# Thefefe/orbit

Hardware: AMD Instinct MI355X
Metric: meshlets_culled_per_sec (higher is better)
Workload: dtype f32

## Files before the change

orbit_amd/csrc/abi_ctx.hip:

```cpp
#include <cstdarg>
#include <cstdio>
#include <cstdlib>

#include "abi_internal.h"

thread_local char g_err[512] = "no error";

int32_t fail(OrbitCtx *ctx, int32_t code, const char *fmt, ...) {
    char buf[512];
    va_list ap;
    va_start(ap, fmt);
    vsnprintf(buf, sizeof(buf), fmt, ap);
    va_end(ap);
    snprintf(g_err, sizeof(g_err), "%s", buf);
    if (ctx) snprintf(ctx->err, sizeof(ctx->err), "%s", buf);
    return code;
}

namespace {

size_t layout_arena(OrbitCtx *ctx, uintptr_t base, uint64_t md32) {
    const OrbitCaps &caps = ctx->caps;
    const size_t ent = align_up((size_t)caps.max_entities, 256);
    const size_t mtiles = ((size_t)md32 + kTileRecords - 1) / kTileRecords + 1;
    const size_t cchunks = ((size_t)caps.max_clusters / 1024 + 64) * 32;
    size_t off = 0;
    auto carve = [&](size_t bytes) {
        const uintptr_t p = base + off;
        off = align_up(off + bytes, 256);
        return p;
    };
    ctx->status = (int32_t *)carve(256);
    ctx->debug_cycles = (unsigned long long *)carve(256 + 16 * 8192);
    ctx->zero_page = (void *)carve(256);
    ctx->g_counts = (uint32_t *)carve(256);
    ctx->m_tickets = (uint32_t *)carve((kTicketPools + kEmitTicketPools) * kTicketStride * 4);
    ctx->m_list_sync = (uint32_t *)carve(kListSyncWords * 4);
    ctx->f_done = (uint32_t *)carve((size_t)kShardDoneWords * kShardDoneStride * 4);
    ctx->f_sync = (uint32_t *)carve(kFusedSyncWords * 4);
    ctx->f_ent_flags = (uint32_t *)carve((ent / 256 + 2) * 4);
    ctx->d_tickets = (uint32_t *)carve((size_t)kMaxPyramidBatch * kDepthTicketWords * 4);
    ctx->e_proto = (OrbitMeshletDispatch *)carve(ent * sizeof(OrbitMeshletDispatch));
    ctx->e_block_sums = (uint32_t *)carve((ent / 256 + 1) * 4);
    ctx->e_total = (uint32_t *)carve(256);
    ctx->m_tile_counts = (uint32_t *)carve(mtiles * 4);
    ctx->m_tile_base = (uint32_t *)carve(mtiles * 4);
    ctx->m_total = (uint32_t *)carve(256);
    ctx->f_tile_flags = (uint32_t *)carve(((size_t)md32 / 4 + 2) * 4);
    ctx->m_split = ctx->rec_shift > 5u ? (uint8_t *)carve(ORBIT_DISPATCH_HEADER + 16 * (size_t)md32) : nullptr;
    ctx->x_block_pop = (uint32_t *)carve((size_t)kExpandBlocks * 4);
    ctx->m_tile_masks = (uint32_t *)carve(mtiles * 64);
    ctx->m_tile_payload = (Payload *)carve(mtiles * 128 * sizeof(Payload));
    ctx->m_chunk_sums = (uint32_t *)carve((mtiles / kScanChunk + 2) * 4);
    ctx->c_chunk = (uint32_t *)carve((2 * cchunks + 64) * 4);
    ctx->c_chunk_words = cchunks;
    ctx->a_view_lights = (float4 *)carve((size_t)caps.max_lights * 16 + 1024);
    ctx->a_light_flags = (uint32_t *)carve(((size_t)caps.max_lights / 32 + 64) * 4);
    ctx->a_counts = (uint32_t *)carve(((size_t)caps.max_clusters + kAssignPad) * 4);
    ctx->a_block_sums = (uint32_t *)carve((((size_t)caps.max_clusters / kScanChunk + 2) * kChunkSumStride + 64) * 4);
    ctx->a_block_base = (uint32_t *)carve(((size_t)caps.max_clusters + kAssignPad) * 4);
    ctx->a_total = (uint32_t *)carve(256);
    const size_t agroups = (size_t)caps.max_clusters / 256 + 1;
    const size_t aseg = (((size_t)caps.max_lights + 15) / 16 + 63) / 64 * 64;
    ctx->a_aabb = (float *)carve(((size_t)caps.max_clusters + kAssignPad) * 6 * 4);
    ctx->a_coarse = (uint32_t *)carve(agroups * 16 * aseg * 4);
    ctx->a_coarse_lights = (float4 *)carve(agroups * 16 * aseg * 16);
    ctx->a_coarse_counts = (uint32_t *)carve(agroups * 16 * 4);
    ctx->a_group_box = (float *)carve(agroups * 32);
    ctx->a_group_order = (uint32_t *)carve((agroups + 1) * 4);
    ctx->a_coarse_seg = (uint32_t)aseg;
    ctx->a_hit_cache = (uint32_t *)carve(((size_t)caps.max_clusters + kAssignPad) * kHitCache * 4);
// ... 254 lines not shown
```

orbit_amd/csrc/abi_cull.hip:

```cpp
#include "abi_internal.h"

namespace {

int32_t check_cull_info(OrbitCtx *ctx, const OrbitGpuCullInfo *ci) {
    if (!ci) return fail(ctx, ORBIT_E_INVALID, "cull_info is NULL");
    if (ci->cull_plane_count > ORBIT_MAX_CULL_PLANES)
        return fail(ctx, ORBIT_E_PLANES, "cull_plane_count %u > %d", ci->cull_plane_count, ORBIT_MAX_CULL_PLANES);
    if (ci->projection_type > 1) return fail(ctx, ORBIT_E_INVALID, "projection_type %u", ci->projection_type);
    if (ci->occlusion_pass > 2) return fail(ctx, ORBIT_E_INVALID, "occlusion_pass %u", ci->occlusion_pass);
    return ORBIT_OK;
}

MeshSideView mesh_side_for(OrbitMeshletStream *ms, const void *mesh_info_buffer, bool count = true) {
    if (!ms) return MeshSideView{nullptr, 0u};
    std::lock_guard<std::mutex> lock(ms->mu);
    if (ms->mesh_side == nullptr || ms->mesh_source != mesh_info_buffer || ms->mesh_hi == 0u) return MeshSideView{nullptr, 0u};
    if (count) ms->mesh_side_culls++;
    return MeshSideView{ms->mesh_side, ms->mesh_hi};
}

PyramidView make_pyramid_view(const float *texels, const uint32_t size[2],
                              const OrbitDepthPyramidLevel *levels = nullptr) {
    PyramidView v;
    v.texels = texels;
// ... 349 lines not shown
    PreparedCullViews pc;
    const int32_t rc = prepare_cull_views(ctx, views, count, 0u, pc);
    if (rc != ORBIT_OK) return rc;
    return launch_prepared_cull_views(ctx, pc, (hipStream_t)stream);
}

int32_t orbit_cull_shard(OrbitCtx *ctx, const OrbitGpuCullInfo *ci, const OrbitEntityCullBufs *eb, uint32_t draw_first,
                         uint32_t draw_count, const OrbitMeshletCullBufs *mb, void *record_buffer,
                         uint32_t record_capacity, uint32_t with_commands, void *stream) {
    if (!ctx) return fail(nullptr, ORBIT_E_INVALID, "ctx is NULL");
    std::lock_guard<std::mutex> lock(ctx->mu);
    if (ctx->rec_shift != 5u)
        return fail(ctx, ORBIT_E_INVALID, "cull_shard: the sharded engine's record list is defined for dispatch_size 32; this "
                                          "context has %u", ctx->caps.dispatch_size);
    const hipStream_t s = (hipStream_t)stream;
    const MeshletCullOut out{MeshletCullOut::kRecordList, record_buffer, record_capacity, with_commands ? "cull_shard" : nullptr};
    EntityCullParams ep;
    MeshletCullParams p;
    int32_t rc = entity_cull_params(ctx, ctx, ci, eb, draw_first, draw_count, true, ep);
    if (rc == ORBIT_OK) rc = meshlet_cull_params(ctx, ctx, ci, mb, out, p);
    if (rc != ORBIT_OK) return rc;
    if (mb->meshlet_dispatch_buffer != eb->meshlet_dispatch_buffer)
        return fail(ctx, ORBIT_E_INVALID, "cull_shard: the meshlet stage must read the entity stage's dispatch buffer");
    hipEvent_t ev0, ev1;
    rc = profile_pair(ctx, ev0, ev1);
    if (rc == ORBIT_OK) rc = validate_stream(ctx, p, s);
    if (rc == ORBIT_OK) rc = validate_mesh_side(ctx, ep, s);
    if (rc != ORBIT_OK) return rc;
    const uint32_t chunks = (draw_count + 255u) / 256u;
    const bool one_launch = ci->occlusion_pass == 0u && chunks >= 1u && chunks <= kShardMaxChunks && ctx->caps.cull_path != 1u;
    hipError_t e;
    if (one_launch) {
        FusedCullParams f = fused_params(ep, p, ctx, chunks);
        f.done_flags = ctx->f_done;
        if (ev0 && (e = hipEventRecord(ev0, s)) != hipSuccess) return hip_fail(ctx, e, "hipEventRecord");
        e = launch_shard_cull(f, ctx->num_cus, s);
        if (e != hipSuccess) return hip_fail(ctx, e, "launch shard_cull");
        if (ev1 && (e = hipEventRecord(ev1, s)) != hipSuccess) return hip_fail(ctx, e, "hipEventRecord");
        if (with_commands) {
            MeshletCullParams c = p;
            c.visible_list = 0u;
            c.draw_buffer = p.also_commands;
            c.draw_capacity = p.also_commands_capacity;
            e = launch_meshlet_scan_emit(c, ctx->num_cus, s);
            if (e != hipSuccess) return hip_fail(ctx, e, "launch scan + emit");
        }
        ctx->shard_culls++;
    } else {
        e = launch_entity_cull(ep, draw_count, ctx->num_cus, s);
        if (e != hipSuccess) return hip_fail(ctx, e, "launch entity_cull");
        e = launch_meshlet_cull(p, ctx->num_cus, s, ev0, ev1);
        if (e != hipSuccess) return hip_fail(ctx, e, "launch meshlet_cull");
    }
    count_stream_cull(ctx, p);
    return ORBIT_OK;
}

int32_t orbit_expand_visible_records(OrbitCtx *ctx, const void *record_buffer, const void *meshlet_buffer,
                                     void *draw_commands_buffer, uint32_t draw_capacity, void *stream) {
    if (!ctx) return fail(nullptr, ORBIT_E_INVALID, "ctx is NULL");
    std::lock_guard<std::mutex> lock(ctx->mu);
    if (!record_buffer || !meshlet_buffer || !draw_commands_buffer)
        return fail(ctx, ORBIT_E_MISSING, "expand_visible_records: NULL argument");
    const MeshletStreamView view = stream_view_for(ctx->meshlet_stream, meshlet_buffer, nullptr);
    if (view.sphere && ctx->caps.validate_streams)
        (void)launch_meshlet_stream_validate((const OrbitMeshlet *)meshlet_buffer, view, nullptr, 0, ctx->status,
                                             (hipStream_t)stream);
// ... 71 lines not shown
```

orbit_amd/csrc/abi_internal.h:

```cpp
#pragma once
#include <hip/hip_runtime.h>

#include <atomic>
#include <cstdint>
#include <cstring>
#include <mutex>
#include <new>
#include <vector>

#include "kernels.h"

using namespace orbit;

#pragma GCC visibility push(hidden)

struct OrbitMeshletStream {
    int device = 0;
    uint64_t first = 0, capacity = 0;
    uint4 *sphere = nullptr;
    uint32_t *cone = nullptr;
    uint16_t *mat = nullptr;
    uint32_t *cmd = nullptr;
    uint16_t *cnt = nullptr;
    uint32_t *link = nullptr, *cls0 = nullptr, *cls1 = nullptr;
// ... 7 lines not shown
    hipEvent_t other_event = nullptr;
    bool other_pending = false;
    bool other_recorded = false;
    std::atomic<int> bindings{0};
    MeshSide *mesh_side = nullptr;
    uint32_t mesh_capacity = 0, mesh_hi = 0;
    const void *mesh_source = nullptr;
    uint64_t mesh_side_culls = 0;
};

struct OrbitCtx {
    int device = 0;
    uint32_t num_cus = 0;
    OrbitCaps caps{};
    std::mutex mu;
    uint8_t *arena = nullptr;
    size_t arena_bytes = 0;
    OrbitMeshletDispatch *e_proto = nullptr;
    uint32_t *e_block_sums = nullptr, *e_total = nullptr;
    Payload *m_tile_payload = nullptr;
    uint32_t *m_tile_masks = nullptr, *m_chunk_sums = nullptr;
    uint32_t *m_tile_counts = nullptr, *m_tile_base = nullptr, *m_total = nullptr;
    uint32_t *s_block_sums = nullptr;
    float *b_mesh_slices = nullptr;
    uint32_t *x_block_pop = nullptr;
    uint32_t *c_chunk = nullptr;
    size_t c_chunk_words = 0;
    float4 *a_view_lights = nullptr, *a_coarse_lights = nullptr;
    uint32_t *a_light_flags = nullptr, *a_counts = nullptr, *a_block_sums = nullptr, *a_block_base = nullptr,
             *a_total = nullptr, *a_coarse = nullptr, *a_coarse_counts = nullptr, *a_hit_cache = nullptr;
    float *a_aabb = nullptr, *a_group_box = nullptr;
    uint32_t *a_group_order = nullptr;
    uint32_t a_coarse_seg = 0;
    uint32_t *m_tickets = nullptr, *m_list_sync = nullptr, *f_done = nullptr;
    uint32_t *f_sync = nullptr, *f_ent_flags = nullptr, *f_tile_flags = nullptr;
    uint32_t *d_tickets = nullptr;
    uint8_t *m_split = nullptr;
    uint32_t rec_shift = 5;
    uint64_t fused_culls = 0;
    uint64_t shard_culls = 0;
    uint32_t *g_counts = nullptr;
    int32_t *status = nullptr;
    uint32_t debug_flags = 0;
    uint32_t scan_patience = 256;
    unsigned long long *debug_cycles = nullptr;
    void *zero_page = nullptr;
    uint32_t profiling = 0;
    uint32_t prof_calls = 0;
    std::vector<hipEvent_t> prof_events;
    size_t prof_used = 0;
    std::vector<OrbitCtx *> view_ctx;
    hipStream_t side_stream[2] = {nullptr, nullptr};
    hipEvent_t side_event[3] = {nullptr, nullptr, nullptr};
    OrbitMeshletStream *meshlet_stream = nullptr;
    uint64_t stream_culls = 0;
    uint64_t class_culls = 0;
    char err[512] = {0};
};

constexpr uint32_t kExpandBlocks = 65536;

constexpr uint32_t kMeshBoundsSlots = 1024;

extern thread_local char g_err[512];

int32_t fail(OrbitCtx *ctx, int32_t code, const char *fmt, ...);

// ... 68 lines not shown
```

orbit_amd/csrc/entity_common.h:

```cpp
#pragma once
#include "handoff.h"

namespace orbit {

namespace {

constexpr int kEntityBlock = 256;

enum : uint32_t { kEntNone = 0, kEntSkipped, kEntFrustum, kEntOcclusion, kEntEarly, kEntDrawn };
struct EntityVerdict {
    uint32_t cls;
    uint32_t lod;
};

template <class P>
__device__ __forceinline__ OrbitMeshletDispatch entity_eval_one(const P &p, uint32_t g, bool active, bool &visible,
                                                                EntityVerdict *verdict = nullptr) {
    const OrbitGpuCullInfo &ci = p.ci;
    const bool meshlet_occ = ci.meshlet_visibility_buffer != ORBIT_NONE;
    visible = false;
    OrbitMeshletDispatch pr = {0u, 0u, 0u, 0u};
    if (verdict) verdict->cls = kEntNone, verdict->lod = 0u;
    if (active) {
        const OrbitEntityDraw *draws =
// ... 105 lines not shown
                const uint32_t mid = (lo[u] + hi[u]) >> 1;
                if (s_off[mid] <= r0 + u * kEntityBlock) lo[u] = mid; else hi[u] = mid;
            }
        }
#pragma unroll
        for (uint32_t u = 0; u < U; u++) {
            const uint32_t r = r0 + u * kEntityBlock;
            if (r < total) store(r, entity_record(s_proto[lo[u]], r - s_off[lo[u]], rec_shift));
        }
    }
}
static_assert(kEntityBlock == 256, "entity_expand_records: eight bisection steps");

struct FusedEntity {
    const OrbitGpuCullInfo &ci;
    const uint8_t *entity_draw_buffer;
    const OrbitMeshInfo *mesh_infos;
    MeshSideView mesh_side;
    const OrbitEntityData *entities;
    uint32_t *visibility;
    PyramidView pyr;
};

struct EntityChunksArgs {
    uint8_t *dispatch_buffer;
    uint32_t dispatch_capacity;
    uint32_t draw_first, draw_limit;
    uint32_t ne_chunks;
    uint32_t rec_shift;
    uint32_t *sync;
    uint32_t *ent_flags;
    uint32_t *total;
    int32_t *status;
};
struct EntityChunksLds {
    uint32_t smem[kEntityBlock / 64 + 1];
    uint32_t off[kEntityBlock];
    OrbitMeshletDispatch proto[kEntityBlock];
    uint32_t word;
};

__device__ __forceinline__ uint32_t chunks_before(int32_t *status, __amdgpu_buffer_rsrc_t EF, uint32_t eb, uint32_t *smem) {
    uint32_t part = 0;
    for (uint32_t j = threadIdx.x; j < eb; j += kEntityBlock) {
        uint32_t v = ld_sc1(EF, j * 4u);
        for (uint32_t spins = 0; v == 0u; spins++) {
            if (spins == kSpinLimit) {
                latch_status(status, ORBIT_E_TIMEOUT);
                break;
            }
            poll_pause();
            v = ld_sc1(EF, j * 4u);
        }
        part += v >> 2;
    }
    const int lane = threadIdx.x & 63, wave = threadIdx.x >> 6;
    const uint32_t w = wave_reduce_add(part);
    __syncthreads();
    if (lane == 0) smem[wave] = w;
    __syncthreads();
    uint32_t sum = 0;
#pragma unroll
    for (uint32_t i = 0; i < kEntityBlock / 64; i++) sum += smem[i];
    __syncthreads();
    return uniform(sum);
}



template <class E, class OnTotal>
__device__ __forceinline__ void entity_chunks(const E &ent, const EntityChunksArgs &a, EntityChunksLds &S, OnTotal on_total) {
    const __amdgpu_buffer_rsrc_t EF = rsrc_of(a.ent_flags, a.ne_chunks * 4u);
    const __amdgpu_buffer_rsrc_t REC_W = rsrc_of(a.dispatch_buffer + ORBIT_DISPATCH_HEADER, a.dispatch_capacity * 16u);
    const uint32_t draw_count = *reinterpret_cast<const uint32_t *>(ent.entity_draw_buffer);
    const uint32_t draw_end = min(draw_count, a.draw_limit);
    if (threadIdx.x == 0) S.word = ticket(a.sync + kSyEntTicket);
    __syncthreads();
    uint32_t eb = uniform(S.word);
    __syncthreads();
    while (eb < a.ne_chunks) {
        const uint32_t g = a.draw_first + eb * kEntityBlock + threadIdx.x;
        const bool active = g < draw_end;
        bool visible;
        const OrbitMeshletDispatch pr = entity_eval_one(ent, g, active, visible);
        entity_write_visibility(ent, g, draw_end, active && visible);
        const uint32_t n = (pr.meshlet_count + (1u << a.rec_shift) - 1u) >> a.rec_shift;
        uint32_t chunk_total;
        S.off[threadIdx.x] = block_exclusive_scan<kEntityBlock / 64>(n, S.smem, &chunk_total);
        chunk_total = min(uniform(chunk_total), a.dispatch_capacity + 1u);
        S.proto[threadIdx.x] = pr;
        st_sc1(EF, threadIdx.x == 0 ? eb * 4u : kHandoffNoOffset, chunk_total << 2 | kAggregate);
        const uint32_t base = chunks_before(a.status, EF, eb, S.smem);
        entity_expand_records(S.off, S.proto, chunk_total, a.rec_shift, [&](uint32_t r, const OrbitMeshletDispatch &rec) {
            const v4u w = {rec.entity_index, rec.meshlet_offset, rec.meshlet_count, rec.visibility_offset};
            const uint64_t slot = (uint64_t)base + r;
            __builtin_amdgcn_raw_buffer_store_b128(w, REC_W, slot < a.dispatch_capacity ? (uint32_t)slot * 16u : kHandoffNoOffset, 0, kSc1);
        });
        drain_stores();
        __syncthreads();
        if (threadIdx.x == 0) {
            const unsigned long long before = arrive(a.sync + kSyEntDone, chunk_total);
            if ((uint32_t)(before >> 40) == a.ne_chunks - 1u) {
                const unsigned long long total64 = (before & kArriveRecords) + chunk_total;
                const uint32_t total = total64 > 0xFFFFFFFFull ? 0xFFFFFFFFu : (uint32_t)total64;
                uint32_t *hdr = reinterpret_cast<uint32_t *>(a.dispatch_buffer);
                hdr[0] = min(total, a.dispatch_capacity);
                hdr[1] = 1u;
                hdr[2] = 1u;
                *a.total = total;
                if (total > a.dispatch_capacity) latch_status(a.status, ORBIT_E_CAPACITY);
                on_total(total);
            }
            S.word = ticket(a.sync + kSyEntTicket);
        }
        __syncthreads();
        eb = uniform(S.word);
        __syncthreads();
    }
}

}

}
```

orbit_amd/csrc/kernels.h:

```cpp
#pragma once
#include <hip/hip_runtime.h>
#include <stdint.h>

#include "../../include/orbit_abi_ext.h"
#include "orbit_device.h"

namespace orbit {

constexpr uint32_t kTileRecords = 16;
constexpr uint32_t kTileRows = 8;
constexpr uint32_t kTicketPools = 8;
constexpr uint32_t kTicketStride = 64;
constexpr uint32_t kEmitTicketPools = 16;
constexpr uint32_t kListGroups = 32;
constexpr uint32_t kListSyncStride = 32;
constexpr uint32_t kListSyncWords = (kListGroups + 1) * kListSyncStride;

struct Payload {
    uint32_t y, z, w;
};

struct MeshSide {
    float sphere[4];
    uint32_t lod_count, lod0_offset, lod0_count, valid;
// ... 132 lines not shown
    float *aabb;
    uint32_t *coarse;
    float4 *coarse_lights;
    uint32_t *coarse_counts;
    float *group_box;
    uint32_t *group_order;
    uint32_t coarse_seg;
    uint32_t *block_sums;
    uint32_t *block_base;
    uint32_t *total;
    uint32_t *zero_words;
    uint32_t zero_count;
    int32_t *status;
    unsigned long long *debug_tests;
};

constexpr uint32_t kSyEntTicket = 0, kSyEntDone = 32, kSyTileTicket = 96, kSyBlocksDone = 128;
constexpr uint32_t kFusedSyncWords = 160;
constexpr uint32_t kFusedMaxEntityDraws = 16384;
struct FusedCullParams {
    MeshletCullParams m;
    const uint8_t *entity_draw_buffer;
    const OrbitMeshInfo *mesh_infos;
    MeshSideView mesh_side;
    uint32_t *visibility;
    PyramidView e_pyr;
    uint32_t draw_first, draw_limit;
    uint32_t e_dispatch_capacity;
    uint32_t ne_chunks;
    uint32_t *e_total;
    uint32_t *sync;
    uint32_t *ent_flags;
    uint32_t *tile_flags;
    uint32_t *done_flags;
};
struct FusedCullViews {
    FusedCullParams v[ORBIT_MAX_CULL_VIEWS];
};
hipError_t launch_cull_fused_views(const FusedCullViews &all, const uint32_t *entity_draw_counts, uint32_t n,
                                   uint32_t num_cus, hipStream_t s);
constexpr uint32_t kShardMaxChunks = 256;
constexpr uint32_t kShardDoneWords = 64, kShardDoneStride = 32;
hipError_t launch_shard_cull(const FusedCullParams &f, uint32_t num_cus, hipStream_t s);
hipError_t launch_meshlet_scan_emit(const MeshletCullParams &p, uint32_t num_cus, hipStream_t s);

hipError_t launch_entity_cull(const EntityCullParams &p, uint32_t entity_draw_count, uint32_t num_cus, hipStream_t s);
struct SplitRecordsParams {
    const uint8_t *src;
    uint8_t *dst;
    uint32_t src_capacity;
    uint32_t rec_shift;
};
struct SplitRecordsViews {
    SplitRecordsParams v[ORBIT_MAX_CULL_VIEWS];
};
hipError_t launch_split_records(const SplitRecordsParams &p, hipStream_t s);
hipError_t launch_split_records_views(const SplitRecordsViews &all, uint32_t n, hipStream_t s);

struct EntityCullViews {
    EntityCullParams v[ORBIT_MAX_CULL_VIEWS];
};
struct MeshletCullViews;
struct FusedCullViews;
struct ViewGroup;
#if !ORBIT_CONTRACT
hipError_t launch_entity_cull_contracted(const EntityCullParams &p, uint32_t entity_draw_count, uint32_t num_cus, hipStream_t s);
hipError_t launch_entity_cull_views_contracted(const EntityCullViews &all, uint32_t n, uint32_t max_entity_draw_count,
                                               uint32_t num_cus, hipStream_t s);
hipError_t launch_meshlet_eval_contracted(const MeshletCullParams &p, uint32_t num_cus, hipStream_t s);
hipError_t launch_meshlet_eval_views_contracted(const MeshletCullViews &all, const ViewGroup &g, uint32_t m, uint32_t pass,
                                                bool ortho, int src, uint32_t max_tiles, uint32_t num_cus, hipStream_t s);
hipError_t launch_shard_cull_contracted(const FusedCullParams &f, uint32_t num_cus, hipStream_t s);
hipError_t launch_cull_fused_views_contracted(const FusedCullViews &all, const uint32_t *entity_draw_counts, uint32_t n,
                                              uint32_t num_cus, hipStream_t s);
#endif
// ... 103 lines not shown
```

orbit_amd/csrc/meshlet_common.h:

```cpp
#pragma once
#include <type_traits>

#include "kernels.h"
#include "scan.h"

namespace orbit {

namespace {

constexpr uint32_t kPayloadCap = 128;

constexpr uint32_t kBufFlags = 0x00020000u;
constexpr uint32_t kNoOffset = 0xFFFFFF00u;

#ifndef ORBIT_EVAL_LOAD_AUX
#define ORBIT_EVAL_LOAD_AUX 2
#endif
#ifndef ORBIT_EMIT_CNT_AUX
#define ORBIT_EMIT_CNT_AUX 2
#endif
#ifndef ORBIT_EMIT_STORE_AUX
#define ORBIT_EMIT_STORE_AUX 0
#endif
struct StreamRsrc {
// ... 454 lines not shown
        L.r[rid].scale = sqrtf(gmax(d0, gmax(d1, d2)));
        L.r[rid].rec = rec;
        L.r[rid].prev = prev_word;
    }
    {
        const bool okc = col == 3 ? (o[3] == 1.0f && o[0] * 0.0f == 0.0f && o[1] * 0.0f == 0.0f && o[2] * 0.0f == 0.0f)
                                  : o[3] == 0.0f;
        uint64_t m = __ballot(okc);
        m &= m >> 1;
        m &= m >> 2;
        m &= m >> 4;
        if (lane == 0) L.affine_rows = m;
    }
    if (lane < (int)kTileRows) L.draw_mask[lane] = 0ull, L.vis_mask[lane] = 0ull;
    __builtin_amdgcn_fence(__ATOMIC_RELEASE, "wavefront");
    __builtin_amdgcn_wave_barrier();
    __builtin_amdgcn_fence(__ATOMIC_ACQUIRE, "wavefront");
}

__device__ __forceinline__ void tile_records_out(const MeshletCullParams &p, const WaveTileLds &L, uint32_t nrec, uint32_t tile,
                                                 uint32_t survivors, uint32_t *wave_sum, int lane) {
    const __amdgpu_buffer_rsrc_t list =
        __builtin_amdgcn_make_buffer_rsrc(p.draw_buffer + ORBIT_VISIBLE_HEADER, 0, min(nrec, p.draw_capacity) * 12u, kBufFlags);
    if (lane == 0) *wave_sum += survivors;
    const uint32_t r = (uint32_t)lane / 3u, k = (uint32_t)lane - 3u * r;
    const uint32_t rr = r < kTileRecords ? r : 0u;
    const uint4 rec = L.r[rr].rec;
    const uint32_t m = reinterpret_cast<const uint32_t *>(L.draw_mask)[rr];
    const uint32_t v = k == 0u ? rec.x : (k == 1u ? rec.y : m);
    const uint32_t off = lane < (int)(3u * kTileRecords) ? tile * (kTileRecords * 12u) + (uint32_t)lane * 4u : kNoOffset;
    __builtin_amdgcn_raw_buffer_store_b32(v, list, off, 0, 0);
}

template <int WAVES>
__device__ __forceinline__ void records_finish(const MeshletCullParams &p, uint32_t nrec, const uint32_t *s_red,
                                               uint32_t *ent_flags = nullptr, uint32_t ne_chunks = 0u, uint32_t *sync = nullptr,
                                               uint32_t *done_flags = nullptr) {
    asm volatile("s_waitcnt vmcnt(0)" ::: "memory");
    __syncthreads();
    if (threadIdx.x != 0) return;
    unsigned long long sum = 0;
#pragma unroll
    for (int w = 0; w < WAVES; w++) sum += s_red[w];
    constexpr unsigned long long kOne = 1ull << 40, kSum = kOne - 1ull;
    unsigned long long *sy = reinterpret_cast<unsigned long long *>(p.list_sync);
    const uint32_t g = blockIdx.x % kListGroups;
    const uint32_t in_group = (gridDim.x - g + kListGroups - 1u) / kListGroups;
    const unsigned long long a = __hip_atomic_fetch_add(sy + g * (kListSyncStride / 2u), kOne | sum, __ATOMIC_RELAXED, __HIP_MEMORY_SCOPE_AGENT);
    if ((uint32_t)(a >> 40) != in_group - 1u) return;
    const unsigned long long group_sum = (a & kSum) + sum;
    const uint32_t groups = min(gridDim.x, kListGroups);
    const unsigned long long t = __hip_atomic_fetch_add(sy + kListGroups * (kListSyncStride / 2u), kOne | group_sum, __ATOMIC_RELAXED, __HIP_MEMORY_SCOPE_AGENT);
    if ((uint32_t)(t >> 40) != groups - 1u) return;
    const unsigned long long total = (t & kSum) + group_sum;
    for (uint32_t k = 0; k <= kListGroups; k++) sy[k * (kListSyncStride / 2u)] = 0ull;
    uint32_t *hdr = reinterpret_cast<uint32_t *>(p.draw_buffer);
    hdr[0] = min(nrec, p.draw_capacity);
    hdr[1] = (uint32_t)total;
    *p.total = nrec;
    if (nrec > p.draw_capacity) latch_status(p.status, ORBIT_E_CAPACITY);
    for (uint32_t q = 0; q < kTicketPools; q++) p.tickets[q * kTicketStride] = 0u;
    if (ent_flags != nullptr) {
        for (uint32_t i = 0; i < ne_chunks; i++) ent_flags[i] = 0u;
        for (uint32_t i = 0; i < kFusedSyncWords; i++) sync[i] = 0u;
        for (uint32_t k = 0; k < kShardDoneWords; k++) done_flags[k * kShardDoneStride] = 0u, done_flags[k * kShardDoneStride + 1u] = 0u;
    }
}

#ifdef ORBIT_TRIAGE
#define ORBIT_DBG(p, bits) (((p).debug_flags & (bits)) != 0u)
#else
#define ORBIT_DBG(p, bits) false
#endif

}

}
```

orbit_amd/csrc/meshlet_eval.hip:

```cpp
#include "entity_common.h"
#include "meshlet_common.h"

namespace orbit {

namespace {

constexpr int kEvWaves = 4;
constexpr int kEvWavesPerSimd = 4;
#ifndef ORBIT_EV_WPS0
#define ORBIT_EV_WPS0 5
#endif
constexpr int ev_waves_per_simd(int pass, bool stream) { return (pass == 0 && stream) ? ORBIT_EV_WPS0 : kEvWavesPerSimd; }


__device__ __forceinline__ void clear_chunk_sums(const MeshletCullParams &p) {
    if (blockIdx.x != 0) return;
    const uint32_t max_tiles = (p.dispatch_capacity + kTileRecords - 1) / kTileRecords;
    const uint32_t max_chunks = (max_tiles + kScanChunk - 1) / kScanChunk;
    for (uint32_t c = threadIdx.x; c < max_chunks; c += kEvWaves * 64) p.chunk_sums[c] = 0u;
    if (threadIdx.x < kEmitTicketPools) p.tickets[(kTicketPools + threadIdx.x) * kTicketStride] = 0u;
}

constexpr uint32_t kShardPatience = 256;

template <bool FUSED>
__device__ __forceinline__ uint4 eval_load_rec(const MeshletCullParams &p, uint32_t tile, bool tile_valid, uint32_t nrec, int lane) {
    if constexpr (FUSED) {
        const __amdgpu_buffer_rsrc_t R = rsrc_of(p.dispatch_buffer + ORBIT_DISPATCH_HEADER, nrec * 16u);
        const uint32_t rec_index = tile * kTileRecords + (uint32_t)(lane >> 2);
        const auto w = __builtin_amdgcn_raw_buffer_load_b128(R, (tile_valid && rec_index < nrec) ? rec_index * 16u : kNoOffset, 0, kSc1);
        return make_uint4(w[0], w[1], w[2], w[3]);
    } else {
        return setup_load_rec(p, tile, tile_valid, nrec, lane);
    }
}

template <int PASS, int PROJ, bool PROF, bool STREAM = false, bool CLS = false, bool LIST = false, bool FUSED = false>
__device__ __forceinline__ void meshlet_eval_body(const MeshletCullParams &p, const FusedCullParams *fp = nullptr) {
    static_assert(!FUSED || LIST, "the shard launch writes the record list");
    __shared__ std::conditional_t<FUSED, EntityChunksLds, uint32_t> ent_lds;
    __shared__ uint32_t s_word[2];
    __shared__ WaveTileLds lds[kEvWaves][3];
    __shared__ PlaneLds planes;
    __shared__ AlphaLds alpha_tab;
    __shared__ CandLds<(PASS == 2 ? kCandRing : 1u)> cand_ring[kEvWaves];
    const int lane = threadIdx.x & 63, wave = threadIdx.x >> 6;
#ifdef ORBIT_TRIAGE
    const unsigned long long wall_enter = wall_clock64();
    unsigned long long wall_chunks = 0;
#endif
    const bool occ2 = PASS == 2 && p.ci.meshlet_visibility_buffer != ORBIT_NONE;
    __shared__ uint32_t cls_sel[CLS ? 8 : 1];
    __shared__ uint32_t s_red[kEvWaves];
    uint32_t nrec_raw = 0;
    if constexpr (!FUSED) nrec_raw = *reinterpret_cast<const uint32_t *>(p.dispatch_buffer);
    const uint32_t stride = gridDim.x * kEvWaves, wave_g = blockIdx.x * kEvWaves + wave;
    uint4 r0, r1, rec2;
    if constexpr (!FUSED) {
        const uint32_t cap_tiles = (p.dispatch_capacity + kTileRecords - 1) / kTileRecords;
        r0 = setup_load_rec(p, wave_g, wave_g < cap_tiles, p.dispatch_capacity, lane);
        r1 = setup_load_rec(p, wave_g + stride, wave_g + stride < cap_tiles, p.dispatch_capacity, lane);
        rec2 = setup_load_rec(p, wave_g + 2u * stride, wave_g + 2u * stride < cap_tiles, p.dispatch_capacity, lane);
    }
    planes_to_lds(p, planes);
    clear_chunk_sums(p);
    if (threadIdx.x < kEvWaves) s_red[threadIdx.x] = 0u;
    if (CLS && threadIdx.x < 6) cls_sel[threadIdx.x] = ((alpha_bits(p.ci, threadIdx.x >> 1) >> (threadIdx.x & 1u)) & 1u) ? ~0u : 0u;
    const AlphaLds *alpha = alpha_table_fill(p, alpha_tab) ? &alpha_tab : nullptr;
    __syncthreads();
    if constexpr (FUSED) {
        const FusedCullParams &f = *fp;
        const FusedEntity E{p.ci, f.entity_draw_buffer, f.mesh_infos, f.mesh_side, p.entities, f.visibility, f.e_pyr};
        EntityChunksArgs a;
        a.dispatch_buffer = const_cast<uint8_t *>(p.dispatch_buffer);
        a.dispatch_capacity = f.e_dispatch_capacity;
        a.draw_first = f.draw_first, a.draw_limit = f.draw_limit;
        a.ne_chunks = f.ne_chunks;
        a.rec_shift = 5u;
        a.sync = f.sync, a.ent_flags = f.ent_flags, a.total = f.e_total, a.status = p.status;
        const __amdgpu_buffer_rsrc_t DN = rsrc_of(f.done_flags, kShardDoneWords * kShardDoneStride * 4u);
        auto tell_all = [&](uint32_t total) {
            typedef unsigned int v2u __attribute__((ext_vector_type(2)));
            const v2u v = {total, 1u << 8};
            for (uint32_t k = 0; k < kShardDoneWords; k++)
                __builtin_amdgcn_raw_buffer_store_b64(v, DN, k * kShardDoneStride * 4u, 0, kSc1);
        };
        if (blockIdx.x < f.ne_chunks) entity_chunks(E, a, ent_lds, tell_all);
#ifdef ORBIT_TRIAGE
        wall_chunks = wall_clock64();
#endif
        const uint32_t my_copy = (blockIdx.x % kShardDoneWords) * kShardDoneStride * 4u;
        for (uint32_t round = 0;; round++) {
            if (threadIdx.x == 0) {
                if (round == 0u && blockIdx.x >= f.ne_chunks) asm volatile("s_sleep 64" ::: "memory");
                auto w = __builtin_amdgcn_raw_buffer_load_b64(DN, my_copy, 0, kSc1);
                for (uint32_t spins = 0; arrived_chunks(w) == 0u && spins < kShardPatience; spins++) {
                    asm volatile("s_sleep 8" ::: "memory");
                    w = __builtin_amdgcn_raw_buffer_load_b64(DN, my_copy, 0, kSc1);
                }
                s_word[0] = arrived_chunks(w) != 0u ? 1u : 0u;
                s_word[1] = arrived_records(w);
            }
            __syncthreads();
            const uint32_t done = uniform(s_word[0]);
            nrec_raw = uniform(s_word[1]);
            __syncthreads();
            if (done != 0u) break;
            if (round == kSpinLimit / kShardPatience) {
                if (threadIdx.x == 0) latch_status(p.status, ORBIT_E_TIMEOUT);
                nrec_raw = 0u;
                break;
            }
            entity_chunks(E, a, ent_lds, tell_all);
        }
        nrec_raw = min(nrec_raw, f.e_dispatch_capacity);
    }
    const uint32_t nrec = min(nrec_raw, p.dispatch_capacity);
    const uint32_t ntiles = (nrec + kTileRecords - 1) / kTileRecords;
    const bool static_share = ORBIT_DBG(p, 64u);
    const uint32_t full_rounds = ntiles / stride;
    const uint32_t dyn_rounds = ORBIT_DBG(p, 256u) ? 2u : ORBIT_DBG(p, 512u) ? 4u : ORBIT_DBG(p, 1024u) ? 1u : min(max(full_rounds / 4u, 1u), 3u);
    const uint32_t n_static = (static_share || ntiles <= stride) ? 0xFFFFFFFFu : (ORBIT_DBG(p, 128u) ? 3u : max(full_rounds >= dyn_rounds ? full_rounds - dyn_rounds : 0u, 3u));
    const uint32_t npools = min((uint32_t)kTicketPools, stride);
    const uint32_t pool = wave_g % npools;
    uint32_t *ticket_ctr = p.tickets + pool * kTicketStride;
    uint32_t claims = 0;
    auto claim = [&]() -> uint32_t {
        uint32_t raw = claims;
        if (claims >= n_static) {
            raw = 0;
            if (lane == 0) raw = atomicAdd(ticket_ctr, 1u);
        }
        claims++;
        return raw;
    };
    auto ticket_tile = [&](uint32_t raw, uint32_t k) -> uint32_t {
        const uint32_t t = (uint32_t)__builtin_amdgcn_readfirstlane((int)raw);
        if (k < n_static) return t * stride + wave_g;
        return t >= 0x08000000u ? 0xFFFFFFFFu : n_static * stride + t * npools + pool;
    };
    StreamRsrc SR = {};
    if constexpr (STREAM) {
        SR.first = p.ms.first;
        SR.count = p.ms.count;
        SR.sphere = __builtin_amdgcn_make_buffer_rsrc(const_cast<uint4 *>(p.ms.sphere + p.ms.first), 0, p.ms.count * 16u, kBufFlags);
        SR.cone = __builtin_amdgcn_make_buffer_rsrc(const_cast<uint32_t *>(p.ms.cone + p.ms.first), 0, p.ms.count * 4u, kBufFlags);
        if constexpr (!CLS)
            SR.mat = __builtin_amdgcn_make_buffer_rsrc(const_cast<uint16_t *>(p.ms.mat + p.ms.first), 0, p.ms.count * 2u, kBufFlags);
    }
    uint32_t w0, w1, w2, tk_raw;
    {
        const uint32_t t0 = claim(), t1 = claim(), t2 = claim();
        tk_raw = claim();
        w0 = ticket_tile(t0, 0u);
        w1 = ticket_tile(t1, 1u);
        w2 = ticket_tile(t2, 2u);
    }
    RowRegs<1> qa, qb;
    {
        if constexpr (FUSED) {
            r0 = eval_load_rec<true>(p, w0, w0 < ntiles, nrec, lane);
            r1 = eval_load_rec<true>(p, w1, w1 < ntiles, nrec, lane);
            rec2 = eval_load_rec<true>(p, w2, w2 < ntiles, nrec, lane);
        } else {
            const uint4 none = make_uint4(0u, 0u, 0u, 0u);
            const uint32_t rl = (uint32_t)lane >> 2;
            if (!(w0 < ntiles && w0 * kTileRecords + rl < nrec)) r0 = none;
            if (!(w1 < ntiles && w1 * kTileRecords + rl < nrec)) r1 = none;
            if (!(w2 < ntiles && w2 * kTileRecords + rl < nrec)) rec2 = none;
        }
        if ((lane & 3) == 0) lds[wave][0].r[lane >> 2].rec = r0;
        __builtin_amdgcn_fence(__ATOMIC_RELEASE, "wavefront");
        __builtin_amdgcn_wave_barrier();
        __builtin_amdgcn_fence(__ATOMIC_ACQUIRE, "wavefront");
        const float4 m0 = setup_load_mat(p, r0, lane);
        const float4 m1 = setup_load_mat(p, r1, lane);
        uint32_t c0 = 0u, c1 = 0u;
        if constexpr (CLS) c0 = setup_load_cls(p, r0, lane), c1 = setup_load_cls(p, r1, lane);
        rows_load<PASS, 0, 1, STREAM, CLS>(p, lds[wave][0], lane, qa, &SR);
        rows_load<PASS, 1, 1, STREAM, CLS>(p, lds[wave][0], lane, qb, &SR);
        if constexpr (CLS) {
            setup_write_cls(lds[wave][0], cls_sel, r0, c0, lane);
            setup_write_cls(lds[wave][1], cls_sel, r1, c1, lane);
        }
        setup_write(p, lds[wave][0], r0, m0, lane);
        setup_write(p, lds[wave][1], r1, m1, lane);
    }
    uint32_t it = 0;
#ifdef ORBIT_TRIAGE
    unsigned long long tc[6] = {0, 0, 0, 0, 0, 0}, t0 = 0, t1;
#define EV_STAMP(k)                            \
    if (PROF && !(p.debug_flags & 16u)) {      \
        t1 = __builtin_amdgcn_s_memtime();     \
        __builtin_amdgcn_s_waitcnt(0xC07F);    \
        tc[k] += t1 - t0;                      \
        t0 = t1;                               \
    }
    unsigned long long wall_begin = 0;
    if (p.debug_flags & 16u) wall_begin = (p.debug_flags & 2048u) ? wall_enter : (p.debug_flags & 4096u) ? wall_chunks : wall_clock64();
    if (PROF) {
        t0 = __builtin_amdgcn_s_memtime();
        __builtin_amdgcn_s_waitcnt(0xC07F);
    }
// ... 38 lines not shown
        uint32_t cls2 = 0u;
        if constexpr (CLS) cls2 = setup_load_cls(p, rec2, lane);
        const uint4 rec3 = eval_load_rec<FUSED>(p, w3, w3 < ntiles, nrec, lane);
        EV_STAMP(1)
        EV_ROW(4, qa)
        rows_load<PASS, 6, 1, STREAM, CLS>(p, L, lane, qa, &SR);
        EV_ROW(5, qb)
        rows_load<PASS, 7, 1, STREAM, CLS>(p, L, lane, qb, &SR);
        EV_STAMP(2)
        EV_ROW(6, qa)
        rows_load<PASS, 0, 1, STREAM, CLS>(p, Ln, lane, qa, &SR);
        EV_ROW(7, qb)
        rows_load<PASS, 1, 1, STREAM, CLS>(p, Ln, lane, qb, &SR);
        EV_STAMP(3)
        if constexpr (PASS == 2) {
            if (occ2) tile_finish_occ(p, L, cand_ring[wave], lane, cs, payload);
        }
#undef EV_ROW
        if constexpr (CLS) setup_write_cls(lds[wave][(it + 2) % 3], cls_sel, rec2, cls2, lane);
        setup_write(p, lds[wave][(it + 2) % 3], rec2, mat2, lane);
        const bool rec_list = LIST && p.visible_list == 2u;
        if (((STREAM && !(rec_list && p.also_commands == nullptr)) || p.task_records != nullptr || cs.total > kPayloadCap) && lane < 2 * (int)kTileRows)
            p.tile_masks[(size_t)w0 * (2 * kTileRows) + lane] = reinterpret_cast<const uint32_t *>(L.draw_mask)[lane];
        if (lane == 0) p.tile_counts[w0] = cs.total;
        if (rec_list) tile_records_out(p, L, nrec, w0, cs.total, s_red + wave, lane);
        EV_STAMP(4)
        w0 = w1;
        w1 = w2;
        w2 = w3;
        rec2 = rec3;
        it++;
    }
#undef EV_STAMP
    if constexpr (FUSED) records_finish<kEvWaves>(p, nrec, s_red, fp->ent_flags, fp->ne_chunks, fp->sync, fp->done_flags);
    else if (LIST && p.visible_list == 2u) records_finish<kEvWaves>(p, nrec, s_red);
#ifdef ORBIT_TRIAGE
    if (PROF && lane == 0) {
        for (int k = 0; k < 5; k++) atomicAdd(p.debug_cycles + k, tc[k]);
        atomicAdd(p.debug_cycles + 7, 1ull);
    }
    if ((p.debug_flags & 16u) && lane == 0) {
        const uint32_t wg = blockIdx.x * kEvWaves + wave;
        if (wg < 8192u) {
            p.debug_cycles[32 + 2 * wg] = wall_begin;
            p.debug_cycles[32 + 2 * wg + 1] = wall_clock64();
        }
    }
#endif
}

template <int PASS, int PROJ, bool PROF, bool STREAM = false, bool CLS = false>
__global__ __launch_bounds__(kEvWaves * 64, ev_waves_per_simd(PASS, STREAM)) void meshlet_eval_kernel(const MeshletCullParams p) {
    meshlet_eval_body<PASS, PROJ, PROF, STREAM, CLS>(p);
}
template <int PASS, int PROJ, bool STREAM, bool CLS = false>
__global__ __launch_bounds__(kEvWaves * 64, ev_waves_per_simd(PASS, STREAM)) void meshlet_eval_views_kernel(const MeshletCullViews all,
                                                                                           const ViewGroup g) {
    meshlet_eval_body<PASS, PROJ, false, STREAM, CLS, true>(all.v[g.idx[blockIdx.y]]);
}

struct ShardCullArgs {
    FusedCullParams v[2];
};
template <int PROJ, bool STREAM, bool CLS>
__global__ __launch_bounds__(kEvWaves * 64, kEvWavesPerSimd) void shard_cull_kernel(const ShardCullArgs all, const ViewGroup g) {
    const FusedCullParams &f = all.v[g.idx[blockIdx.y] & 1u];
    meshlet_eval_body<0, PROJ, false, STREAM, CLS, true, true>(f.m, &f);
}

struct Pass1Item {
    uint4 a, b;
    uint32_t code;
};

__device__ __forceinline__ uint32_t pass1_load_prev(const MeshletCullParams &p, const uint4 &rec, int lane) {
    const bool rw_vis = p.ci.meshlet_visibility_buffer != ORBIT_NONE;
    const uint32_t *src = (rw_vis && rec.z != 0u && (lane & 3) == 0) ? p.meshlet_visibility + rec.w
                                                                    : reinterpret_cast<const uint32_t *>(p.zero_page);
// ... 298 lines not shown
```

Measured before the change: 193.2 billion.

## Replace shard done-flag handoff with per-chunk stored prefixes for early meshlet start

In the fused shard cull, entity chunks used to signal completion by writing a single total to replicated done words, and meshlet blocks waited until every chunk had finished. Each entity chunk now publishes its running record prefix into replicated per-chunk slots. Meshlet blocks poll these with a wave-wide 128-bit load and start loading their first tiles as soon as the records they need are covered, so entity and meshlet work overlap. The cost is more complex polling, several sync points per block, and a parallel reset of the larger stored-prefix array at the end.

```diff
diff --git a/orbit_amd/csrc/abi_ctx.hip b/orbit_amd/csrc/abi_ctx.hip
--- a/orbit_amd/csrc/abi_ctx.hip
+++ b/orbit_amd/csrc/abi_ctx.hip
@@ -36,7 +36,7 @@
     ctx->g_counts = (uint32_t *)carve(256);
     ctx->m_tickets = (uint32_t *)carve((kTicketPools + kEmitTicketPools) * kTicketStride * 4);
     ctx->m_list_sync = (uint32_t *)carve(kListSyncWords * 4);
-    ctx->f_done = (uint32_t *)carve((size_t)kShardDoneWords * kShardDoneStride * 4);
+    ctx->f_stored = (uint32_t *)carve((size_t)kShardStoredCopies * kShardMaxChunks * 4);
     ctx->f_sync = (uint32_t *)carve(kFusedSyncWords * 4);
     ctx->f_ent_flags = (uint32_t *)carve((ent / 256 + 2) * 4);
     ctx->d_tickets = (uint32_t *)carve((size_t)kMaxPyramidBatch * kDepthTicketWords * 4);
diff --git a/orbit_amd/csrc/abi_cull.hip b/orbit_amd/csrc/abi_cull.hip
--- a/orbit_amd/csrc/abi_cull.hip
+++ b/orbit_amd/csrc/abi_cull.hip
@@ -405,7 +405,7 @@
     hipError_t e;
     if (one_launch) {
         FusedCullParams f = fused_params(ep, p, ctx, chunks);
-        f.done_flags = ctx->f_done;
+        f.ent_stored = ctx->f_stored;
         if (ev0 && (e = hipEventRecord(ev0, s)) != hipSuccess) return hip_fail(ctx, e, "hipEventRecord");
         e = launch_shard_cull(f, ctx->num_cus, s);
         if (e != hipSuccess) return hip_fail(ctx, e, "launch shard_cull");
diff --git a/orbit_amd/csrc/abi_internal.h b/orbit_amd/csrc/abi_internal.h
--- a/orbit_amd/csrc/abi_internal.h
+++ b/orbit_amd/csrc/abi_internal.h
@@ -63,7 +63,7 @@
     float *a_aabb = nullptr, *a_group_box = nullptr;
     uint32_t *a_group_order = nullptr;
     uint32_t a_coarse_seg = 0;
-    uint32_t *m_tickets = nullptr, *m_list_sync = nullptr, *f_done = nullptr;
+    uint32_t *m_tickets = nullptr, *m_list_sync = nullptr, *f_stored = nullptr;
     uint32_t *f_sync = nullptr, *f_ent_flags = nullptr, *f_tile_flags = nullptr;
     uint32_t *d_tickets = nullptr;
     uint8_t *m_split = nullptr;
diff --git a/orbit_amd/csrc/entity_common.h b/orbit_amd/csrc/entity_common.h
--- a/orbit_amd/csrc/entity_common.h
+++ b/orbit_amd/csrc/entity_common.h
@@ -161,6 +161,7 @@
     uint32_t *ent_flags;
     uint32_t *total;
     int32_t *status;
+    uint32_t *ent_stored = nullptr;
 };
 struct EntityChunksLds {
     uint32_t smem[kEntityBlock / 64 + 1];
@@ -200,6 +201,7 @@
 template <class E, class OnTotal>
 __device__ __forceinline__ void entity_chunks(const E &ent, const EntityChunksArgs &a, EntityChunksLds &S, OnTotal on_total) {
     const __amdgpu_buffer_rsrc_t EF = rsrc_of(a.ent_flags, a.ne_chunks * 4u);
+    const __amdgpu_buffer_rsrc_t ES = rsrc_of(a.ent_stored, a.ent_stored != nullptr ? kShardStoredCopies * kShardMaxChunks * 4u : 0u);
     const __amdgpu_buffer_rsrc_t REC_W = rsrc_of(a.dispatch_buffer + ORBIT_DISPATCH_HEADER, a.dispatch_capacity * 16u);
     const uint32_t draw_count = *reinterpret_cast<const uint32_t *>(ent.entity_draw_buffer);
     const uint32_t draw_end = min(draw_count, a.draw_limit);
@@ -227,6 +229,11 @@
         });
         drain_stores();
         __syncthreads();
+        if (a.ent_stored != nullptr) {
+            const unsigned long long prefix64 = (unsigned long long)base + chunk_total;
+            const uint32_t prefix = prefix64 > a.dispatch_capacity ? a.dispatch_capacity + 1u : (uint32_t)prefix64;
+            st_sc1(ES, threadIdx.x < kShardStoredCopies ? (threadIdx.x * kShardMaxChunks + eb) * 4u : kHandoffNoOffset, prefix << 1 | 1u);
+        }
         if (threadIdx.x == 0) {
             const unsigned long long before = arrive(a.sync + kSyEntDone, chunk_total);
             if ((uint32_t)(before >> 40) == a.ne_chunks - 1u) {
diff --git a/orbit_amd/csrc/kernels.h b/orbit_amd/csrc/kernels.h
--- a/orbit_amd/csrc/kernels.h
+++ b/orbit_amd/csrc/kernels.h
@@ -188,7 +188,7 @@
     uint32_t *sync;
     uint32_t *ent_flags;
     uint32_t *tile_flags;
-    uint32_t *done_flags;
+    uint32_t *ent_stored;
 };
 struct FusedCullViews {
     FusedCullParams v[ORBIT_MAX_CULL_VIEWS];
@@ -196,7 +196,7 @@
 hipError_t launch_cull_fused_views(const FusedCullViews &all, const uint32_t *entity_draw_counts, uint32_t n,
                                    uint32_t num_cus, hipStream_t s);
 constexpr uint32_t kShardMaxChunks = 256;
-constexpr uint32_t kShardDoneWords = 64, kShardDoneStride = 32;
+constexpr uint32_t kShardStoredCopies = 32;
 hipError_t launch_shard_cull(const FusedCullParams &f, uint32_t num_cus, hipStream_t s);
 hipError_t launch_meshlet_scan_emit(const MeshletCullParams &p, uint32_t num_cus, hipStream_t s);
 
diff --git a/orbit_amd/csrc/meshlet_common.h b/orbit_amd/csrc/meshlet_common.h
--- a/orbit_amd/csrc/meshlet_common.h
+++ b/orbit_amd/csrc/meshlet_common.h
@@ -510,26 +510,20 @@
     __builtin_amdgcn_raw_buffer_store_b32(v, list, off, 0, 0);
 }
 
-template <int WAVES>
-__device__ __forceinline__ void records_finish(const MeshletCullParams &p, uint32_t nrec, const uint32_t *s_red,
-                                               uint32_t *ent_flags = nullptr, uint32_t ne_chunks = 0u, uint32_t *sync = nullptr,
-                                               uint32_t *done_flags = nullptr) {
-    asm volatile("s_waitcnt vmcnt(0)" ::: "memory");
-    __syncthreads();
-    if (threadIdx.x != 0) return;
+__device__ __forceinline__ bool records_arrive(const MeshletCullParams &p, uint32_t nrec, const uint32_t *s_red, int waves) {
     unsigned long long sum = 0;
 #pragma unroll
-    for (int w = 0; w < WAVES; w++) sum += s_red[w];
+    for (int w = 0; w < waves; w++) sum += s_red[w];
     constexpr unsigned long long kOne = 1ull << 40, kSum = kOne - 1ull;
     unsigned long long *sy = reinterpret_cast<unsigned long long *>(p.list_sync);
     const uint32_t g = blockIdx.x % kListGroups;
     const uint32_t in_group = (gridDim.x - g + kListGroups - 1u) / kListGroups;
     const unsigned long long a = __hip_atomic_fetch_add(sy + g * (kListSyncStride / 2u), kOne | sum, __ATOMIC_RELAXED, __HIP_MEMORY_SCOPE_AGENT);
-    if ((uint32_t)(a >> 40) != in_group - 1u) return;
+    if ((uint32_t)(a >> 40) != in_group - 1u) return false;
     const unsigned long long group_sum = (a & kSum) + sum;
     const uint32_t groups = min(gridDim.x, kListGroups);
     const unsigned long long t = __hip_atomic_fetch_add(sy + kListGroups * (kListSyncStride / 2u), kOne | group_sum, __ATOMIC_RELAXED, __HIP_MEMORY_SCOPE_AGENT);
-    if ((uint32_t)(t >> 40) != groups - 1u) return;
+    if ((uint32_t)(t >> 40) != groups - 1u) return false;
     const unsigned long long total = (t & kSum) + group_sum;
     for (uint32_t k = 0; k <= kListGroups; k++) sy[k * (kListSyncStride / 2u)] = 0ull;
     uint32_t *hdr = reinterpret_cast<uint32_t *>(p.draw_buffer);
@@ -538,11 +532,27 @@
     *p.total = nrec;
     if (nrec > p.draw_capacity) latch_status(p.status, ORBIT_E_CAPACITY);
     for (uint32_t q = 0; q < kTicketPools; q++) p.tickets[q * kTicketStride] = 0u;
-    if (ent_flags != nullptr) {
-        for (uint32_t i = 0; i < ne_chunks; i++) ent_flags[i] = 0u;
-        for (uint32_t i = 0; i < kFusedSyncWords; i++) sync[i] = 0u;
-        for (uint32_t k = 0; k < kShardDoneWords; k++) done_flags[k * kShardDoneStride] = 0u, done_flags[k * kShardDoneStride + 1u] = 0u;
-    }
+    return true;
+}
+template <int WAVES>
+__device__ __forceinline__ void records_finish(const MeshletCullParams &p, uint32_t nrec, uint32_t *s_red,
+                                               uint32_t *ent_flags = nullptr, uint32_t ne_chunks = 0u, uint32_t *sync = nullptr,
+                                               uint32_t *ent_stored = nullptr) {
+    asm volatile("s_waitcnt vmcnt(0)" ::: "memory");
+    __syncthreads();
+    if (ent_flags == nullptr) {
+        if (threadIdx.x == 0) (void)records_arrive(p, nrec, s_red, WAVES);
+        return;
+    }
+    if (threadIdx.x == 0) s_red[0] = records_arrive(p, nrec, s_red, WAVES) ? 1u : 0u;
+    __syncthreads();
+    if (__builtin_amdgcn_readfirstlane((int)s_red[0]) == 0) return;
+    const uint32_t nthreads = WAVES * 64u;
+    for (uint32_t i = threadIdx.x; i < ne_chunks; i += nthreads) ent_flags[i] = 0u;
+    for (uint32_t i = threadIdx.x; i < kFusedSyncWords; i += nthreads) sync[i] = 0u;
+    const uint32_t quads = (ne_chunks + 3u) / 4u;
+    for (uint32_t i = threadIdx.x; i < kShardStoredCopies * quads; i += nthreads)
+        reinterpret_cast<uint4 *>(ent_stored + (i / quads) * kShardMaxChunks)[i % quads] = make_uint4(0u, 0u, 0u, 0u);
 }
 
 #ifdef ORBIT_TRIAGE
diff --git a/orbit_amd/csrc/meshlet_eval.hip b/orbit_amd/csrc/meshlet_eval.hip
--- a/orbit_amd/csrc/meshlet_eval.hip
+++ b/orbit_amd/csrc/meshlet_eval.hip
@@ -47,7 +47,7 @@
     const int lane = threadIdx.x & 63, wave = threadIdx.x >> 6;
 #ifdef ORBIT_TRIAGE
     const unsigned long long wall_enter = wall_clock64();
-    unsigned long long wall_chunks = 0;
+    unsigned long long wall_chunks = 0, wall_first_row = 0;
 #endif
     const bool occ2 = PASS == 2 && p.ci.meshlet_visibility_buffer != ORBIT_NONE;
     __shared__ uint32_t cls_sel[CLS ? 8 : 1];
@@ -68,6 +68,19 @@
     if (CLS && threadIdx.x < 6) cls_sel[threadIdx.x] = ((alpha_bits(p.ci, threadIdx.x >> 1) >> (threadIdx.x & 1u)) & 1u) ? ~0u : 0u;
     const AlphaLds *alpha = alpha_table_fill(p, alpha_tab) ? &alpha_tab : nullptr;
     __syncthreads();
+    auto stream_rsrc = [&]() {
+        StreamRsrc R = {};
+        if constexpr (STREAM) {
+            R.first = p.ms.first;
+            R.count = p.ms.count;
+            R.sphere = __builtin_amdgcn_make_buffer_rsrc(const_cast<uint4 *>(p.ms.sphere + p.ms.first), 0, p.ms.count * 16u, kBufFlags);
+            R.cone = __builtin_amdgcn_make_buffer_rsrc(const_cast<uint32_t *>(p.ms.cone + p.ms.first), 0, p.ms.count * 4u, kBufFlags);
+            if constexpr (!CLS)
+                R.mat = __builtin_amdgcn_make_buffer_rsrc(const_cast<uint16_t *>(p.ms.mat + p.ms.first), 0, p.ms.count * 2u, kBufFlags);
+        }
+        return R;
+    };
+    RowRegs<1> qa, qb;
     if constexpr (FUSED) {
         const FusedCullParams &f = *fp;
         const FusedEntity E{p.ci, f.entity_draw_buffer, f.mesh_infos, f.mesh_side, p.entities, f.visibility, f.e_pyr};
@@ -78,42 +91,84 @@
         a.ne_chunks = f.ne_chunks;
         a.rec_shift = 5u;
         a.sync = f.sync, a.ent_flags = f.ent_flags, a.total = f.e_total, a.status = p.status;
-        const __amdgpu_buffer_rsrc_t DN = rsrc_of(f.done_flags, kShardDoneWords * kShardDoneStride * 4u);
-        auto tell_all = [&](uint32_t total) {
-            typedef unsigned int v2u __attribute__((ext_vector_type(2)));
-            const v2u v = {total, 1u << 8};
-            for (uint32_t k = 0; k < kShardDoneWords; k++)
-                __builtin_amdgcn_raw_buffer_store_b64(v, DN, k * kShardDoneStride * 4u, 0, kSc1);
-        };
-        if (blockIdx.x < f.ne_chunks) entity_chunks(E, a, ent_lds, tell_all);
+        a.ent_stored = f.ent_stored;
+        if (blockIdx.x < f.ne_chunks) entity_chunks(E, a, ent_lds, [](uint32_t) {});
 #ifdef ORBIT_TRIAGE
         wall_chunks = wall_clock64();
 #endif
-        const uint32_t my_copy = (blockIdx.x % kShardDoneWords) * kShardDoneStride * 4u;
-        for (uint32_t round = 0;; round++) {
-            if (threadIdx.x == 0) {
-                if (round == 0u && blockIdx.x >= f.ne_chunks) asm volatile("s_sleep 64" ::: "memory");
-                auto w = __builtin_amdgcn_raw_buffer_load_b64(DN, my_copy, 0, kSc1);
-                for (uint32_t spins = 0; arrived_chunks(w) == 0u && spins < kShardPatience; spins++) {
-                    asm volatile("s_sleep 8" ::: "memory");
-                    w = __builtin_amdgcn_raw_buffer_load_b64(DN, my_copy, 0, kSc1);
+        const __amdgpu_buffer_rsrc_t ST = rsrc_of(f.ent_stored, kShardStoredCopies * kShardMaxChunks * 4u);
+        const uint32_t my_copy = (blockIdx.x % kShardStoredCopies) * kShardMaxChunks * 4u;
+        const uint32_t quads = (f.ne_chunks + 3u) / 4u;
+        auto poll_stored = [&](uint32_t &covered, uint32_t &all_in) {
+            const auto w = __builtin_amdgcn_raw_buffer_load_b128(ST, (uint32_t)lane < quads ? my_copy + (uint32_t)lane * 16u : kNoOffset, 0, kSc1);
+            const uint32_t k = w[0] == 0u ? 0u : w[1] == 0u ? 1u : w[2] == 0u ? 2u : w[3] == 0u ? 3u : 4u;
+            const uint32_t last = k == 0u ? 0u : k == 1u ? w[0] : k == 2u ? w[1] : k == 3u ? w[2] : w[3];
+            const uint64_t part = ~__ballot(k == 4u);
+            const uint32_t first = part != 0ull ? (uint32_t)__builtin_ctzll(part) : 63u;
+            const uint32_t k_first = part != 0ull ? (uint32_t)__shfl((int)k, (int)first, 64) : 4u;
+            const uint32_t word = (uint32_t)__shfl((int)last, (int)(k_first != 0u ? first : first - 1u), 64);
+            covered = (k_first != 0u || first != 0u) ? word >> 1 : 0u;
+            all_in = first * 4u + k_first >= f.ne_chunks ? 1u : 0u;
+        };
+        const uint32_t patience = ORBIT_DBG(p, 16384u) ? 0u : kShardPatience;
+        const uint32_t cap_rec = min(f.e_dispatch_capacity, p.dispatch_capacity);
+        uint32_t covered = 0u, all_in = 0u;
+        const bool poller = uniform((uint32_t)wave) == 0u;
+#pragma nounroll
+        for (uint32_t stop = 0; stop < 4u; stop++) {
+            const uint32_t need = stop < 3u ? (blockIdx.x * kEvWaves + stop * stride + kEvWaves) * kTileRecords : 0xFFFFFFFFu;
+            for (uint32_t round = 0; covered < need && all_in == 0u; round++) {
+                if (poller) {
+                    if (stop == 0u && round == 0u && blockIdx.x >= f.ne_chunks) asm volatile("s_sleep 64" ::: "memory");
+                    uint32_t cv, in;
+                    poll_stored(cv, in);
+                    for (uint32_t spins = 0; cv < need && in == 0u && spins < patience; spins++) {
+                        asm volatile("s_sleep 8" ::: "memory");
+                        poll_stored(cv, in);
+                    }
+                    if (lane == 0) s_word[0] = cv, s_word[1] = in;
                 }
-                s_word[0] = arrived_chunks(w) != 0u ? 1u : 0u;
-                s_word[1] = arrived_records(w);
+                __syncthreads();
+                covered = uniform(s_word[0]);
+                all_in = uniform(s_word[1]);
+                __syncthreads();
+                if (covered >= need || all_in != 0u) break;
+                if (round == kSpinLimit / max(patience, 1u)) {
+                    if (threadIdx.x == 0) latch_status(p.status, ORBIT_E_TIMEOUT);
+                    covered = 0u, all_in = 1u;
+                    break;
+                }
+                entity_chunks(E, a, ent_lds, [](uint32_t) {});
             }
-            __syncthreads();
-            const uint32_t done = uniform(s_word[0]);
-            nrec_raw = uniform(s_word[1]);
-            __syncthreads();
-            if (done != 0u) break;
-            if (round == kSpinLimit / kShardPatience) {
-                if (threadIdx.x == 0) latch_status(p.status, ORBIT_E_TIMEOUT);
-                nrec_raw = 0u;
-                break;
+            const uint32_t bound = min(covered, cap_rec);
+            const uint32_t tile = wave_g + stop * stride;
+            if (stop == 0u) {
+                r0 = eval_load_rec<true>(p, tile, true, bound, lane);
+                if ((lane & 3) == 0) lds[wave][0].r[lane >> 2].rec = r0;
+                wave_lds_fence();
+                const float4 m0 = setup_load_mat(p, r0, lane);
+                uint32_t c0 = 0u;
+                if constexpr (CLS) c0 = setup_load_cls(p, r0, lane);
+                const StreamRsrc SR0 = stream_rsrc();
+                rows_load<0, 0, 1, STREAM, CLS>(p, lds[wave][0], lane, qa, &SR0);
+                rows_load<0, 1, 1, STREAM, CLS>(p, lds[wave][0], lane, qb, &SR0);
+#ifdef ORBIT_TRIAGE
+                wall_first_row = wall_clock64();
+#endif
+                if constexpr (CLS) setup_write_cls(lds[wave][0], cls_sel, r0, c0, lane);
+                setup_write(p, lds[wave][0], r0, m0, lane);
+            } else if (stop == 1u) {
+                r1 = eval_load_rec<true>(p, tile, true, bound, lane);
+                const float4 m1 = setup_load_mat(p, r1, lane);
+                uint32_t c1 = 0u;
+                if constexpr (CLS) c1 = setup_load_cls(p, r1, lane);
+                if constexpr (CLS) setup_write_cls(lds[wave][1], cls_sel, r1, c1, lane);
+                setup_write(p, lds[wave][1], r1, m1, lane);
+            } else if (stop == 2u) {
+                rec2 = eval_load_rec<true>(p, tile, true, bound, lane);
             }
-            entity_chunks(E, a, ent_lds, tell_all);
-        }
-        nrec_raw = min(nrec_raw, f.e_dispatch_capacity);
+        }
+        nrec_raw = min(covered, f.e_dispatch_capacity);
     }
     const uint32_t nrec = min(nrec_raw, p.dispatch_capacity);
     const uint32_t ntiles = (nrec + kTileRecords - 1) / kTileRecords;
@@ -139,15 +194,7 @@
         if (k < n_static) return t * stride + wave_g;
         return t >= 0x08000000u ? 0xFFFFFFFFu : n_static * stride + t * npools + pool;
     };
-    StreamRsrc SR = {};
-    if constexpr (STREAM) {
-        SR.first = p.ms.first;
-        SR.count = p.ms.count;
-        SR.sphere = __builtin_amdgcn_make_buffer_rsrc(const_cast<uint4 *>(p.ms.sphere + p.ms.first), 0, p.ms.count * 16u, kBufFlags);
-        SR.cone = __builtin_amdgcn_make_buffer_rsrc(const_cast<uint32_t *>(p.ms.cone + p.ms.first), 0, p.ms.count * 4u, kBufFlags);
-        if constexpr (!CLS)
-            SR.mat = __builtin_amdgcn_make_buffer_rsrc(const_cast<uint16_t *>(p.ms.mat + p.ms.first), 0, p.ms.count * 2u, kBufFlags);
-    }
+    const StreamRsrc SR = stream_rsrc();
     uint32_t w0, w1, w2, tk_raw;
     {
         const uint32_t t0 = claim(), t1 = claim(), t2 = claim();
@@ -156,19 +203,12 @@
         w1 = ticket_tile(t1, 1u);
         w2 = ticket_tile(t2, 2u);
     }
-    RowRegs<1> qa, qb;
-    {
-        if constexpr (FUSED) {
-            r0 = eval_load_rec<true>(p, w0, w0 < ntiles, nrec, lane);
-            r1 = eval_load_rec<true>(p, w1, w1 < ntiles, nrec, lane);
-            rec2 = eval_load_rec<true>(p, w2, w2 < ntiles, nrec, lane);
-        } else {
-            const uint4 none = make_uint4(0u, 0u, 0u, 0u);
-            const uint32_t rl = (uint32_t)lane >> 2;
-            if (!(w0 < ntiles && w0 * kTileRecords + rl < nrec)) r0 = none;
-            if (!(w1 < ntiles && w1 * kTileRecords + rl < nrec)) r1 = none;
-            if (!(w2 < ntiles && w2 * kTileRecords + rl < nrec)) rec2 = none;
-        }
+    if constexpr (!FUSED) {
+        const uint4 none = make_uint4(0u, 0u, 0u, 0u);
+        const uint32_t rl = (uint32_t)lane >> 2;
+        if (!(w0 < ntiles && w0 * kTileRecords + rl < nrec)) r0 = none;
+        if (!(w1 < ntiles && w1 * kTileRecords + rl < nrec)) r1 = none;
+        if (!(w2 < ntiles && w2 * kTileRecords + rl < nrec)) rec2 = none;
         if ((lane & 3) == 0) lds[wave][0].r[lane >> 2].rec = r0;
         __builtin_amdgcn_fence(__ATOMIC_RELEASE, "wavefront");
         __builtin_amdgcn_wave_barrier();
@@ -273,7 +313,7 @@
         it++;
     }
 #undef EV_STAMP
-    if constexpr (FUSED) records_finish<kEvWaves>(p, nrec, s_red, fp->ent_flags, fp->ne_chunks, fp->sync, fp->done_flags);
+    if constexpr (FUSED) records_finish<kEvWaves>(p, nrec, s_red, fp->ent_flags, fp->ne_chunks, fp->sync, fp->ent_stored);
     else if (LIST && p.visible_list == 2u) records_finish<kEvWaves>(p, nrec, s_red);
 #ifdef ORBIT_TRIAGE
     if (PROF && lane == 0) {
@@ -284,7 +324,7 @@
         const uint32_t wg = blockIdx.x * kEvWaves + wave;
         if (wg < 8192u) {
             p.debug_cycles[32 + 2 * wg] = wall_begin;
-            p.debug_cycles[32 + 2 * wg + 1] = wall_clock64();
+            p.debug_cycles[32 + 2 * wg + 1] = (FUSED && (p.debug_flags & 8192u)) ? wall_first_row : wall_clock64();
         }
     }
 #endif
```

Result: no change. 193.6 billion, median of 6 (+0.2%).
